# bliunlpr/Robust_e2e_gan

Measured on NVIDIA B200. Metric: utterances/sec (joint step fwd/bwd), higher is better.
Workload: dtype fp32

## Files before the change

robust_e2e_gan_b200/csrc/attloc_loop.cu:

```cuda
#include <math_constants.h>

#include "attloc_common.cuh"
#include "tc_common.cuh"

namespace re2e {
namespace {

#ifdef RE2E_ATT_DEBUG
__device__ long long g_loop_dbg[2][16 * 512];
#define LOOP_DBG_DECL                                                  \
  __shared__ long long dbg_acc[16];                                    \
  if (threadIdx.x == 0)                                                \
    for (int i_ = 0; i_ < 16; ++i_) dbg_acc[i_] = 0;                   \
  long long dbg_last = clock64()
#define LOOP_MARK(slot)                                              \
  do {                                                               \
    if (threadIdx.x == 0) {                                          \
      const long long t_ = clock64();                                \
      dbg_acc[slot] += t_ - dbg_last;                                \
      dbg_last = t_;                                                 \
    }                                                                \
  } while (0)
#define LOOP_DBG_FLUSH(which)                                                                   \
  do {                                                                                          \
    if (threadIdx.x == 0)                                                                       \
      for (int i_ = 0; i_ < 16; ++i_) g_loop_dbg[which][blockIdx.x * 16 + i_] = dbg_acc[i_];    \
  } while (0)
#else
#define LOOP_DBG_DECL
#define LOOP_MARK(slot)
#define LOOP_DBG_FLUSH(which)
#endif

__device__ __forceinline__ void cp_async4(void *dst_smem, const void *src_gmem) {
  asm volatile("cp.async.ca.shared.global [%0], [%1], 4;" ::"r"(smem_u32(dst_smem)), "l"(src_gmem) : "memory");
}
__device__ __forceinline__ void cp_async_commit() { asm volatile("cp.async.commit_group;" ::: "memory"); }
__device__ __forceinline__ void cp_async_wait_all() { asm volatile("cp.async.wait_group 0;" ::: "memory"); }

__device__ __forceinline__ void warp_reduce10(float (&v)[10], int lane) {
  {
    const bool up = lane & 16;
#pragma unroll
    for (int i = 0; i < 5; ++i) {
      const float send = up ? v[i] : v[i + 5], keep = up ? v[i + 5] : v[i];
      v[i] = keep + __shfl_xor_sync(0xffffffffu, send, 16);
    }
  }
  {
    const bool up = lane & 8;
#pragma unroll
    for (int i = 0; i < 2; ++i) {
      const float send = up ? v[i] : v[i + 3], keep = up ? v[i + 3] : v[i];
      v[i] = keep + __shfl_xor_sync(0xffffffffu, send, 8);
    }
    v[2] += __shfl_xor_sync(0xffffffffu, v[2], 8);
  }
  {
    const bool up = lane & 4;
    const float send = up ? v[0] : v[1], keep = up ? v[1] : v[0];
    v[0] = keep + __shfl_xor_sync(0xffffffffu, send, 4);
    v[2] += __shfl_xor_sync(0xffffffffu, v[2], 4);
  }
  {
    const bool up = lane & 2;
    const float send = up ? v[0] : v[2], keep = up ? v[2] : v[0];
    v[0] = keep + __shfl_xor_sync(0xffffffffu, send, 2);
  }
  v[0] += __shfl_xor_sync(0xffffffffu, v[0], 1);
}

constexpr int kLP = 8;
constexpr int kLW = 2 * kLP;
constexpr int kLT = kLW * 32;
constexpr int kLMaxCL = 8;
constexpr int kKG = 12;

struct LoopGeom {
  int tloc_max, App, CKp, Thp, Dp;
  int col_enc, ncols;
};

struct LoopFwdParams {
  const float *pre, *enc, *dec_proj, *att_init, *W_att, *W_conv, *gvec, *gvec_b;
  float scaling;
  float *c_all, *w_all, *conv_all;
  int S, B, Th, D, A, C, K;
  LoopGeom g;
};

struct LoopBwdParams {
  const float *pre, *enc, *dec_proj, *att_init, *w_all, *conv_all, *dc_all, *dw_all, *W_att, *W_conv, *gvec;
  float scaling;
  float *d_pre, *d_decproj, *acc_slots;
  int slot_stride;
  int S, B, Th, D, A, C, K;
  LoopGeom g;
};

template <int APL, int CP, int DPL>
__global__ void __launch_bounds__(kLT, 1) attloc_loop_fwd_kernel(const LoopFwdParams p) {
  constexpr int NT = kLT;
  constexpr int WP = CP + 1;
  constexpr int CPP = (CP + 3) & ~3;
  extern __shared__ __align__(128) unsigned char smraw[];
  const LoopGeom g = p.g;
  const int C = CP == 10 ? 10 : p.C;
  const int Th = p.Th, D = p.D, A = p.A, K = p.K, S = p.S, B = p.B, filts = (p.K - 1) / 2;
  const int tid = threadIdx.x, lane = tid & 31, warp = tid >> 5, half = warp & 1, pair = warp >> 1;
  const int CL = (int)cluster_nctarank(), rank = (int)cluster_ctarank();
  const int b = blockIdx.x / CL;
  const int t0 = min(Th, rank * g.tloc_max), t1 = min(Th, t0 + g.tloc_max), tloc = t1 - t0;
  const int nch = (tloc + kLP - 1) / kLP;
  const int Dp = g.Dp, Dh = (D + 1) / 2;

  uint64_t *full = reinterpret_cast<uint64_t *>(smraw);
  uint64_t *xbar = full + 1;
  uint64_t *tbar = xbar + 2;
  float *tile = reinterpret_cast<float *>(smraw + 128);
  float *app = tile + (size_t)g.tloc_max * (A + D);
  float *wc_s = app + g.App;
  float *watt_s = wc_s + g.CKp;
  float *convp = watt_s + A * WP;
  float *conv_s = convp + round4(kKQ * g.tloc_max * CP);
  float *e_all = conv_s + g.tloc_max * CPP;
  float *epart = e_all + 2 * g.Thp;
  float *cred = epart + round4(2 * g.tloc_max);
  float *cbuf = cred + kLP * Dp;

  const uint32_t xbytes = (uint32_t)Th * 4u + (rank == 0 ? (uint32_t)CL * (uint32_t)D * 4u : 0u);
  if (tid == 0) {
    mbar_init(full, 1);
    mbar_init(&xbar[0], 1);
    mbar_init(&xbar[1], 1);
    mbar_init(tbar, 1);
    mbar_fence_init();
    mbar_expect_tx(&xbar[0], xbytes);
    mbar_expect_tx(&xbar[1], xbytes);
    if (rank == 0) mbar_expect_tx(tbar, (uint32_t)CL * (uint32_t)D * 4u);
  }
  cluster_arrive_relaxed();
  float gv[APL];
#pragma unroll
  for (int j = 0; j < APL; ++j) gv[j] = __ldg(p.gvec + half * (A / 2) + lane + 32 * j);
  const float gb = __ldg(p.gvec_b);
  for (int i = tid; i < C * K; i += NT) wc_s[i] = __ldg(p.W_conv + i);
  for (int i = tid; i < A * C; i += NT) { const int a = i / C; watt_s[a * WP + (i - a * C)] = __ldg(p.W_att + i); }
  pdl_wait();
  if (tid == 0 && tloc > 0) {
    mbar_expect_tx(full, (uint32_t)tloc * (uint32_t)(A + D) * 4u);
    bulk_g2s(tile, p.pre + ((size_t)b * Th + t0) * A, (uint32_t)tloc * A * 4u, full);
    bulk_g2s(tile + (size_t)g.tloc_max * A, p.enc + ((size_t)b * Th + t0) * D, (uint32_t)tloc * D * 4u, full);
  }
  for (int i = tid; i < g.App; i += NT) {
    const int t = i - filts;
    app[i] = (t >= 0 && t < Th) ? __ldg(p.att_init + (size_t)b * Th + t) : 0.0f;
  }
  __syncthreads();
  constexpr int APH = (APL + 1) / 2;
  float2 WattP[APH][CP];
#pragma unroll
  for (int jp = 0; jp < APH; ++jp) {
    const int a0 = half * (A / 2) + lane + 32 * (2 * jp), a1 = a0 + 32;
#pragma unroll
    for (int c = 0; c < CP; ++c)
      WattP[jp][c] = make_float2(c < C ? watt_s[a0 * WP + c] : 0.0f, (c < C && 2 * jp + 1 < APL) ? watt_s[a1 * WP + c] : 0.0f);
  }
  uint32_t dmask = 0;
#pragma unroll
  for (int j = 0; j < DPL; ++j)
    if (lane + 32 * j < Dh && half * Dh + lane + 32 * j < D) dmask |= 1u << j;
  const int aoff = half * (A / 2) + lane;
  cluster_wait();
  if (tloc > 0) mbar_wait(full, 0);
  LOOP_DBG_DECL;
  LOOP_MARK(0);

  for (int s = 0; s < S; ++s) {
    const uint32_t par = (uint32_t)s & 1u, ph = ((uint32_t)s >> 1) & 1u;
    float *e_cur = e_all + par * g.Thp;
    float *cb = cbuf + par * kLMaxCL * Dp;
    float dp[APL];
#pragma unroll
    for (int j = 0; j < APL; ++j) dp[j] = __ldg(p.dec_proj + ((size_t)s * B + b) * A + aoff + 32 * j);

    {
      const int ntg = (tloc + kTG - 1) / kTG;
      const int Kq = (K + kKQ - 1) / kKQ;
      const int nitems = ntg * C * kKQ;
      for (int item = tid; item < nitems; item += NT) {
        const int tg = item % ntg, rest = item / ntg, c = rest % C, kq = rest / C;
        const int k0 = kq * Kq, k1 = min(K, k0 + Kq);
        const float *wr = wc_s + c * K;
        const float *ar = app + t0 + kTG * tg;
        float a0 = 0.f, a1 = 0.f, a2 = 0.f, a3 = 0.f, a4 = 0.f;
        float x0 = ar[k0], x1 = ar[k0 + 1], x2 = ar[k0 + 2], x3 = ar[k0 + 3];
#pragma unroll 5
        for (int k = k0; k < k1; ++k) {
          const float x4 = ar[k + 4], wv2 = wr[k];
          a0 = fmaf(wv2, x0, a0); a1 = fmaf(wv2, x1, a1); a2 = fmaf(wv2, x2, a2);
          a3 = fmaf(wv2, x3, a3); a4 = fmaf(wv2, x4, a4);
          x0 = x1; x1 = x2; x2 = x3; x3 = x4;
        }
        float *o = convp + ((size_t)kq * g.tloc_max + kTG * tg) * CP + c;
        const int nv = min(kTG, tloc - kTG * tg);
        o[0] = a0;
        if (nv > 1) o[CP] = a1;
        if (nv > 2) o[2 * CP] = a2;
        if (nv > 3) o[3 * CP] = a3;
        if (nv > 4) o[4 * CP] = a4;
      }
    }
    __syncthreads();
    LOOP_MARK(1);
    for (int i = tid; i < tloc * CPP; i += NT) {
      const int tl = i / CPP, c = i - tl * CPP;
      float v = 0.0f;
      if (c < C) {
#pragma unroll
        for (int kq = 0; kq < kKQ; ++kq) v += convp[((size_t)kq * g.tloc_max + tl) * CP + c];
        if (p.conv_all) p.conv_all[(((size_t)s * B + b) * Th + t0 + tl) * C + c] = v;
      }
      conv_s[i] = v;
    }
    __syncthreads();
    LOOP_MARK(2);

    float acc[DPL];
#pragma unroll
    for (int j = 0; j < DPL; ++j) acc[j] = 0.0f;
#pragma unroll 2
    for (int q = 0; q < nch; ++q) {
      const int tl = kLP * q + pair;
      if (tl < tloc) {
        const float *cvp = conv_s + tl * CPP;
        float cv[CPP];
#pragma unroll
        for (int c4 = 0; c4 < CPP; c4 += 4) {
          const float4 t4 = *reinterpret_cast<const float4 *>(cvp + c4);
          cv[c4] = t4.x; cv[c4 + 1] = t4.y; cv[c4 + 2] = t4.z; cv[c4 + 3] = t4.w;
        }
        const float *row = tile + (size_t)tl * A + aoff;
        const float pw = app[filts + t0 + tl];
        const float *er = tile + (size_t)g.tloc_max * A + (size_t)tl * D + half * Dh + lane;
        float part = 0.0f;
#pragma unroll
        for (int jp = 0; jp < APH; ++jp) {
          const bool two = 2 * jp + 1 < APL;
          float2 u = make_float2(dp[2 * jp] + row[64 * jp], two ? dp[2 * jp + 1] + row[64 * jp + 32] : 0.0f);
#pragma unroll
          for (int c = 0; c < CP; ++c) u = __ffma2_rn(WattP[jp][c], make_float2(cv[c], cv[c]), u);
          part = fmaf(gv[2 * jp], tanh_ex2(u.x), part);
          if (two) part = fmaf(gv[2 * jp + 1], tanh_ex2(u.y), part);
        }
#pragma unroll
        for (int j = 0; j < DPL; ++j)
          if (dmask & (1u << j)) acc[j] = fmaf(pw, er[32 * j], acc[j]);
        part = warp_sum(part);
        if (lane == 0) epart[2 * tl + half] = part;
      }
    }
#pragma unroll
    for (int j = 0; j < DPL; ++j)
      if (dmask & (1u << j)) cred[pair * Dp + half * Dh + lane + 32 * j] = acc[j];
    LOOP_MARK(3);
    __syncthreads();
    LOOP_MARK(4);

    for (int d = tid; d < D; d += NT) {
      float sum = 0.0f;
#pragma unroll
      for (int pr = 0; pr < kLP; ++pr) sum += cred[pr * Dp + d];
      st_async_f32(dsmem_addr(cb + rank * Dp + d, 0u), s > 0 ? sum : 0.0f, dsmem_addr(&xbar[par], 0u));
    }
    for (int i = tid; i < tloc * CL; i += NT) {
      const int r = i / tloc, tl = i - r * tloc;
      const float e = p.scaling * ((epart[2 * tl] + epart[2 * tl + 1]) + gb);
      st_async_f32(dsmem_addr(e_cur + t0 + tl, (uint32_t)r), e, dsmem_addr(&xbar[par], (uint32_t)r));
    }
    LOOP_MARK(5);
    mbar_wait(&xbar[par], ph);
    LOOP_MARK(6);
    float M = -CUDART_INF_F;
    for (int t = lane; t < Th; t += 32) M = fmaxf(M, e_cur[t]);
    M = warp_max(M);
    float Ssum = 0.0f;
    for (int t = lane; t < Th; t += 32) Ssum += __expf(e_cur[t] - M);
    Ssum = warp_sum(Ssum);
    const float inv = 1.0f / Ssum;
    for (int t = tid; t < Th; t += NT) {
      const float w = __expf(e_cur[t] - M) * inv;
      app[filts + t] = w;
      if (t >= t0 && t < t1) p.w_all[((size_t)s * B + b) * Th + t] = w;
    }
    if (rank == 0 && s > 0) {
      for (int d = tid; d < D; d += NT) {
        float sum = 0.0f;
        for (int r = 0; r < CL; ++r) sum += cb[r * Dp + d];
        p.c_all[((size_t)(s - 1) * B + b) * D + d] = sum;
      }
    }
    if (tid == 0) mbar_expect_tx(&xbar[par], xbytes);
    __syncthreads();
    LOOP_MARK(7);
  }
  {
    float acc[DPL];
#pragma unroll
    for (int j = 0; j < DPL; ++j) acc[j] = 0.0f;
    for (int q = 0; q < nch; ++q) {
      const int tl = kLP * q + pair;
      if (tl < tloc) {
        const float pw = app[filts + t0 + tl];
        const float *er = tile + (size_t)g.tloc_max * A + (size_t)tl * D + half * Dh + lane;
#pragma unroll
        for (int j = 0; j < DPL; ++j)
          if (dmask & (1u << j)) acc[j] = fmaf(pw, er[32 * j], acc[j]);
      }
    }
#pragma unroll
    for (int j = 0; j < DPL; ++j)
      if (dmask & (1u << j)) cred[pair * Dp + half * Dh + lane + 32 * j] = acc[j];
    __syncthreads();
    float *cb = cbuf + ((uint32_t)S & 1u) * kLMaxCL * Dp;
    for (int d = tid; d < D; d += NT) {
      float sum = 0.0f;
#pragma unroll
      for (int pr = 0; pr < kLP; ++pr) sum += cred[pr * Dp + d];
      st_async_f32(dsmem_addr(cb + rank * Dp + d, 0u), sum, dsmem_addr(tbar, 0u));
    }
    if (rank == 0) {
      mbar_wait(tbar, 0);
      for (int d = tid; d < D; d += NT) {
        float sum = 0.0f;
        for (int r = 0; r < CL; ++r) sum += cb[r * Dp + d];
        p.c_all[((size_t)(S - 1) * B + b) * D + d] = sum;
      }
    }
  }
  LOOP_DBG_FLUSH(0);
}

template <int N>
__device__ __forceinline__ void tmem_ldn(uint32_t taddr, float *v);
template <>
__device__ __forceinline__ void tmem_ldn<1>(uint32_t taddr, float *v) {
  uint32_t r0;
  asm volatile("tcgen05.ld.sync.aligned.32x32b.x1.b32 {%0}, [%1];" : "=r"(r0) : "r"(taddr));
  v[0] = __uint_as_float(r0);
}
template <>
__device__ __forceinline__ void tmem_ldn<2>(uint32_t taddr, float *v) {
  uint32_t r0, r1;
  asm volatile("tcgen05.ld.sync.aligned.32x32b.x2.b32 {%0, %1}, [%2];" : "=r"(r0), "=r"(r1) : "r"(taddr));
  v[0] = __uint_as_float(r0); v[1] = __uint_as_float(r1);
}
template <>
__device__ __forceinline__ void tmem_ldn<4>(uint32_t taddr, float *v) {
  uint32_t r0, r1, r2, r3;
  asm volatile("tcgen05.ld.sync.aligned.32x32b.x4.b32 {%0, %1, %2, %3}, [%4];"
               : "=r"(r0), "=r"(r1), "=r"(r2), "=r"(r3) : "r"(taddr));
  v[0] = __uint_as_float(r0); v[1] = __uint_as_float(r1); v[2] = __uint_as_float(r2); v[3] = __uint_as_float(r3);
}
template <>
__device__ __forceinline__ void tmem_ldn<8>(uint32_t taddr, float *v) {
  uint32_t r[8];
  asm volatile("tcgen05.ld.sync.aligned.32x32b.x8.b32 {%0, %1, %2, %3, %4, %5, %6, %7}, [%8];"
               : "=r"(r[0]), "=r"(r[1]), "=r"(r[2]), "=r"(r[3]), "=r"(r[4]), "=r"(r[5]), "=r"(r[6]), "=r"(r[7])
               : "r"(taddr));
#pragma unroll
  for (int i = 0; i < 8; ++i) v[i] = __uint_as_float(r[i]);
}
// ... 46 lines not shown
  constexpr int NT = kLT;
  constexpr int WP = CP + 1;
  constexpr int CPP = (CP + 3) & ~3;
  constexpr int CH2 = (CP + 1) / 2;
  extern __shared__ __align__(128) unsigned char smraw[];
  const LoopGeom g = p.g;
  const int C = CP == 10 ? 10 : p.C;
  const int Th = p.Th, D = p.D, A = p.A, K = p.K, S = p.S, B = p.B, filts = (p.K - 1) / 2;
  const int tid = threadIdx.x, lane = tid & 31, warp = tid >> 5, half = warp & 1, pair = warp >> 1;
  const int CL = (int)cluster_nctarank(), rank = (int)cluster_ctarank();
  const int b = blockIdx.x / CL;
  const int t0 = min(Th, rank * g.tloc_max), t1 = min(Th, t0 + g.tloc_max), tloc = t1 - t0;
  const int nchx = (tloc + kLP - 1) / kLP;
  const int nche = (tloc + kLW - 1) / kLW;
  const int nchx_max = (g.tloc_max + kLP - 1) / kLP, nche_max = (g.tloc_max + kLW - 1) / kLW;

  uint64_t *done_x = reinterpret_cast<uint64_t *>(smraw);
  uint64_t *xbar1 = done_x + 1;
  uint64_t *xbar2 = xbar1 + 2;
  uint32_t *tmem_slot = reinterpret_cast<uint32_t *>(xbar2 + 2);
  float *xs = reinterpret_cast<float *>(smraw + 128);
  float *dcvT = xs + (size_t)g.tloc_max * A;
  float *app = dcvT + 2 * CP * g.App;
  float *wc_s = app + g.App;
  float *conv_s = wc_s + g.CKp;
  float *w_s = conv_s + g.tloc_max * CPP;
  float *dwt_s = w_s + round4(g.tloc_max);
  float *de_s = dwt_s + round4(g.tloc_max);
  float *dwn_s = de_s + round4(g.tloc_max);
  float *dcv_p = dwn_s + round4(g.tloc_max);
  float *ddp_w = dcv_p + 2 * g.tloc_max * 16;
  float *scr = ddp_w + kLW * (A / 2);
  float *ddp_x = scr + max(A * WP, round4(kKQ * CP * g.tloc_max));
  float *xch = ddp_x + 2 * kLMaxCL * A;
  float *slot = p.acc_slots + (size_t)blockIdx.x * p.slot_stride;

  const uint32_t x1bytes = (uint32_t)CL * 4u;
  const uint32_t x2bytes = (uint32_t)Th * (uint32_t)C * 4u + (rank == 0 ? (uint32_t)CL * (uint32_t)A * 4u : 0u);
  if (tid == 0) {
    mbar_init(done_x, kLW);
    for (int i = 0; i < 2; ++i) { mbar_init(&xbar1[i], 1); mbar_init(&xbar2[i], 1); }
    mbar_fence_init();
    for (int i = 0; i < 2; ++i) { mbar_expect_tx(&xbar1[i], x1bytes); mbar_expect_tx(&xbar2[i], x2bytes); }
  }
  cluster_arrive_relaxed();
  if (warp == 0) tmem_alloc(tmem_slot, 512);
  float gv[APL];
#pragma unroll
  for (int j = 0; j < APL; ++j) gv[j] = __ldg(p.gvec + half * (A / 2) + lane + 32 * j);
  for (int i = tid; i < C * K; i += NT) wc_s[i] = __ldg(p.W_conv + i);
  for (int i = tid; i < A * C; i += NT) { const int a = i / C; scr[a * WP + (i - a * C)] = __ldg(p.W_att + i); }
  {
    const int padn = g.App - Th;
    for (int i = tid; i < 2 * CP * padn; i += NT) {
      const int c = i / padn, o = i - c * padn;
      dcvT[c * g.App + (o < filts ? o : Th + o)] = 0.0f;
    }
    for (int i = tid; i < g.tloc_max * CPP; i += NT) conv_s[i] = 0.0f;
    for (int i = tid; i < round4(g.tloc_max); i += NT) dwn_s[i] = 0.0f;
  }
  tc_fence_before();
  __syncthreads();
  tc_fence_after();
  const uint32_t tbase = *tmem_slot + ((uint32_t)(32 * (warp & 3)) << 16);
  const uint32_t tcol_pre = tbase + (uint32_t)((warp >> 2) * nchx_max * APL);
  const uint32_t tcol_enc = tbase + (uint32_t)(g.col_enc + (warp >> 2) * nche_max * DPL2);
  float2 WattC[APL][CH2];
#pragma unroll
  for (int j = 0; j < APL; ++j) {
    const int a = half * (A / 2) + lane + 32 * j;
#pragma unroll
    for (int c2 = 0; c2 < CH2; ++c2)
      WattC[j][c2] = make_float2(2 * c2 < C ? scr[a * WP + 2 * c2] : 0.0f, 2 * c2 + 1 < C ? scr[a * WP + 2 * c2 + 1] : 0.0f);
  }
  const int aoff = half * (A / 2) + lane;
  pdl_wait();
  for (int q = 0; q < nchx; ++q) {
    const int tl = kLP * q + pair;
    float v[APL];
#pragma unroll
    for (int j = 0; j < APL; ++j) v[j] = tl < tloc ? __ldg(p.pre + ((size_t)b * Th + t0 + tl) * A + aoff + 32 * j) : 0.0f;
    tmem_store<APL>(tcol_pre + (uint32_t)(q * APL), v);
  }
  for (int q = 0; q < nche; ++q) {
    const int tl = kLW * q + warp;
    float v[DPL2];
#pragma unroll
    for (int j = 0; j < DPL2; ++j)
      v[j] = (tl < tloc && lane + 32 * j < D) ? __ldg(p.enc + ((size_t)b * Th + t0 + tl) * D + lane + 32 * j) : 0.0f;
    tmem_store<DPL2>(tcol_enc + (uint32_t)(q * DPL2), v);
  }
  tmem_wait_st();
  __syncthreads();
  cluster_wait();

  float pacc[kKG];
#pragma unroll
  for (int i = 0; i < kKG; ++i) pacc[i] = 0.0f;
  float dgv[APL];
#pragma unroll
  for (int j = 0; j < APL; ++j) dgv[j] = 0.0f;
  float dgb = 0.0f;
  const int nkg = (K + kKG - 1) / kKG;
  const bool conv_thread = tid >= A && tid - A < C * nkg;
  const int cw_c = conv_thread ? (tid - A) / nkg : 0, cw_kb = conv_thread ? ((tid - A) % nkg) * kKG : 0;
  LOOP_DBG_DECL;
  LOOP_MARK(0);

  for (int it = 0; it < S; ++it) {
    const int s = S - 1 - it;
    const uint32_t par = (uint32_t)it & 1u, ph = ((uint32_t)it >> 1) & 1u;
    float *dcv_cur = dcvT + par * CP * g.App;
    float *ddpx = ddp_x + par * kLMaxCL * A;
    float *xc = xch + par * kLMaxCL;
    const size_t sb = (size_t)s * B + b;
    float dcr[DPL2];
#pragma unroll
    for (int j = 0; j < DPL2; ++j) dcr[j] = (p.dc_all && lane + 32 * j < D) ? __ldg(p.dc_all + sb * D + lane + 32 * j) : 0.0f;
    float dp[APL];
#pragma unroll
    for (int j = 0; j < APL; ++j) dp[j] = __ldg(p.dec_proj + sb * A + aoff + 32 * j);
    for (int i = tid; i < tloc; i += NT) {
      w_s[i] = __ldg(p.w_all + sb * Th + t0 + i);
      dwt_s[i] = dwn_s[i] + (p.dw_all ? __ldg(p.dw_all + sb * Th + t0 + i) : 0.0f);
    }
    for (int i = tid; i < tloc * C; i += NT) {
      const int tl = i / C;
      conv_s[tl * CPP + (i - tl * C)] = __ldg(p.conv_all + (sb * Th + t0) * C + i);
    }
    {
      const float *prev = s == 0 ? p.att_init + (size_t)b * Th : p.w_all + (sb - B) * Th;
      for (int i = tid; i < g.App; i += NT) {
        const int t = i - filts;
        app[i] = (t >= 0 && t < Th) ? __ldg(prev + t) : 0.0f;
      }
    }
    __syncthreads();
    LOOP_MARK(1);

    for (int q = 0; q < nche; ++q) {
      const int tl = kLW * q + warp;
      float ev[DPL2];
      tmem_load<DPL2>(tcol_enc + (uint32_t)(q * DPL2), ev);
      tmem_wait_ld();
      float dot = 0.0f;
#pragma unroll
      for (int j = 0; j < DPL2; ++j) dot = fmaf(dcr[j], ev[j], dot);
      dot = warp_sum(dot);
      if (lane == 0 && tl < tloc) dwt_s[tl] += dot;
    }
    __syncthreads();
    LOOP_MARK(2);
    if (warp == 0) {
      float s1 = 0.0f;
      for (int tl = lane; tl < tloc; tl += 32) s1 = fmaf(w_s[tl], dwt_s[tl], s1);
      s1 = warp_sum(s1);
      if (lane < CL) st_async_f32(dsmem_addr(xc + rank, (uint32_t)lane), s1, dsmem_addr(&xbar1[par], (uint32_t)lane));
    }
    mbar_wait(&xbar1[par], ph);
    float Stot = 0.0f;
    for (int r = 0; r < CL; ++r) Stot += xc[r];
    for (int tl = tid; tl < tloc; tl += NT) de_s[tl] = p.scaling * w_s[tl] * (dwt_s[tl] - Stot);
    if (tid == 0) {
      mbar_expect_tx(&xbar1[par], x1bytes);
      if (it > 0) bulk_wait<0>();
    }
    __syncthreads();
    LOOP_MARK(3);

    float ddp[APL];
#pragma unroll
    for (int j = 0; j < APL; ++j) ddp[j] = 0.0f;
    float pn[APL];
    tmem_load<APL>(tcol_pre, pn);
#pragma unroll 1
    for (int q = 0; q < nchx; ++q) {
      const int tl = kLP * q + pair;
      tmem_wait_ld();
      float pv[APL];
#pragma unroll
      for (int j = 0; j < APL; ++j) {
        asm volatile("" : "+f"(pn[j]));
        pv[j] = pn[j];
      }
      if (q + 1 < nchx) tmem_load<APL>(tcol_pre + (uint32_t)((q + 1) * APL), pn);
      if (tl < tloc) {
        const float de = de_s[tl];
        const float *cvp = conv_s + tl * CPP;
        float cv[CPP];
#pragma unroll
        for (int c4 = 0; c4 < CPP; c4 += 4) {
// ... 34 lines not shown
#pragma unroll
          for (int c = 0; c < 8; ++c) { dcv[2 * c] = dcv2[c].x; dcv[2 * c + 1] = dcv2[c].y; }
          warp_reduce16(dcv, lane);
          if ((lane & 1) == 0) {
            const int ci = ((lane >> 4) & 1) * 8 + ((lane >> 3) & 1) * 4 + ((lane >> 2) & 1) * 2 + ((lane >> 1) & 1);
            dcv_p[(half * g.tloc_max + tl) * 16 + ci] = dcv[0];
          }
        }
      }
    }
    LOOP_MARK(4);
    fence_proxy_async_smem();
    __syncwarp();
    if (lane == 0) mbar_arrive1(done_x);
    if (tid == 0 && tloc > 0) {
      mbar_wait(done_x, (uint32_t)it & 1u);
      float *dst = p.d_pre + ((size_t)b * Th + t0) * A;
      const uint32_t total = (uint32_t)tloc * A * 4u;
      for (uint32_t o = 0; o < total; o += 32768u) {
        const uint32_t nb = total - o < 32768u ? total - o : 32768u;
        if (it > 0) bulk_red_add_s2g(reinterpret_cast<char *>(dst) + o, reinterpret_cast<char *>(xs) + o, nb);
        else bulk_s2g(reinterpret_cast<char *>(dst) + o, reinterpret_cast<char *>(xs) + o, nb);
      }
      bulk_commit();
    }
#pragma unroll
    for (int j = 0; j < APL; ++j) ddp_w[warp * (A / 2) + lane + 32 * j] = ddp[j];
    __syncthreads();
    LOOP_MARK(5);

    for (int item = tid; item < tloc * C; item += NT) {
      const int c = item / tloc, tl = item - c * tloc;
      const float v = dcv_p[tl * 16 + c] + dcv_p[(g.tloc_max + tl) * 16 + c];
      for (int r = 0; r < CL; ++r)
        st_async_f32(dsmem_addr(dcv_cur + c * g.App + filts + t0 + tl, (uint32_t)r), v, dsmem_addr(&xbar2[par], (uint32_t)r));
    }
    for (int a = tid; a < A; a += NT) {
      const int h = a >= A / 2 ? 1 : 0, ai = a - h * (A / 2);
      float sd = 0.0f;
#pragma unroll
      for (int pr = 0; pr < kLP; ++pr) sd += ddp_w[(2 * pr + h) * (A / 2) + ai];
      st_async_f32(dsmem_addr(ddpx + rank * A + a, 0u), sd, dsmem_addr(&xbar2[par], 0u));
    }
    if (warp == kLW - 1) {
      float s2 = 0.0f;
      for (int tl = lane; tl < tloc; tl += 32) s2 += de_s[tl];
      dgb += warp_sum(s2);
    }
    LOOP_MARK(6);
    if (tid < A) {
#pragma unroll 5
      for (int tl = 0; tl < tloc; ++tl) {
        const float dt = xs[(size_t)tl * A + tid];
#pragma unroll
        for (int c4 = 0; c4 < CPP; c4 += 4) {
          const float4 t4 = *reinterpret_cast<const float4 *>(conv_s + tl * CPP + c4);
          if (c4 < CP) pacc[c4] = fmaf(dt, t4.x, pacc[c4]);
          if (c4 + 1 < CP) pacc[c4 + 1] = fmaf(dt, t4.y, pacc[c4 + 1]);
          if (c4 + 2 < CP) pacc[c4 + 2] = fmaf(dt, t4.z, pacc[c4 + 2]);
          if (c4 + 3 < CP) pacc[c4 + 3] = fmaf(dt, t4.w, pacc[c4 + 3]);
        }
      }
    } else if (conv_thread) {
      const float *ar = app + cw_kb;
      float x[kKG];
#pragma unroll
      for (int i = 0; i < kKG - 1; ++i) x[i] = ar[t0 + i];
#pragma unroll 12
      for (int tl = 0; tl < tloc; ++tl) {
        x[kKG - 1] = ar[t0 + tl + kKG - 1];
        const float dv = dcv_p[tl * 16 + cw_c] + dcv_p[(g.tloc_max + tl) * 16 + cw_c];
#pragma unroll
        for (int i = 0; i < kKG; ++i) pacc[i] = fmaf(dv, x[i], pacc[i]);
#pragma unroll
        for (int i = 0; i < kKG - 1; ++i) x[i] = x[i + 1];
      }
    }
    LOOP_MARK(7);
    mbar_wait(&xbar2[par], ph);
    LOOP_MARK(8);
    if (rank == 0) {
      for (int a = tid; a < A; a += NT) {
        float sd = 0.0f;
        for (int r = 0; r < CL; ++r) sd += ddpx[r * A + a];
        p.d_decproj[sb * A + a] = sd;
      }
    }
    if (s > 0) {
      const int nsg = (tloc + kTG - 1) / kTG;
      const int Kq = (K + kKQ - 1) / kKQ;
      const int nitems = nsg * C * kKQ;
      for (int item = tid; item < nitems; item += NT) {
        const int sg = item % nsg, rest = item / nsg, c = rest % C, kq = rest / C;
        const int k0 = kq * Kq, k1 = min(K, k0 + Kq);
        const float *wr = wc_s + c * K;
        const float *dr = dcv_cur + c * g.App + (t0 + kTG * sg) + 2 * filts;
        float a0 = 0.f, a1 = 0.f, a2 = 0.f, a3 = 0.f, a4 = 0.f;
        float x1 = dr[1 - k0], x2 = dr[2 - k0], x3 = dr[3 - k0], x4 = dr[4 - k0];
#pragma unroll 5
        for (int k = k0; k < k1; ++k) {
          const float x0 = dr[-k], wv = wr[k];
          a0 = fmaf(wv, x0, a0); a1 = fmaf(wv, x1, a1); a2 = fmaf(wv, x2, a2);
          a3 = fmaf(wv, x3, a3); a4 = fmaf(wv, x4, a4);
          x4 = x3; x3 = x2; x2 = x1; x1 = x0;
        }
        float *o = scr + ((size_t)(kq * C + c)) * g.tloc_max + kTG * sg;
        const int nv = min(kTG, tloc - kTG * sg);
        o[0] = a0;
        if (nv > 1) o[1] = a1;
        if (nv > 2) o[2] = a2;
        if (nv > 3) o[3] = a3;
        if (nv > 4) o[4] = a4;
      }
    }
    if (tid == 0) mbar_expect_tx(&xbar2[par], x2bytes);
    __syncthreads();
    LOOP_MARK(9);
    if (s > 0) {
      for (int tl = tid; tl < tloc; tl += NT) {
        float sum = 0.0f;
        for (int i = 0; i < kKQ * C; ++i) sum += scr[(size_t)i * g.tloc_max + tl];
        dwn_s[tl] = sum;
      }
    }
    LOOP_MARK(10);
  }

  LOOP_DBG_FLUSH(1);
  if (tid < A) {
#pragma unroll
    for (int c = 0; c < CP; ++c)
      if (c < C) slot[tid * C + c] = pacc[c];
  } else if (conv_thread) {
#pragma unroll
    for (int i = 0; i < kKG; ++i)
      if (cw_kb + i < K) slot[A * C + cw_c * K + cw_kb + i] = pacc[i];
  }
  __syncthreads();
#pragma unroll
  for (int j = 0; j < APL; ++j) ddp_w[warp * (A / 2) + lane + 32 * j] = dgv[j];
  __syncthreads();
  for (int a = tid; a < A; a += NT) {
    const int h = a >= A / 2 ? 1 : 0, ai = a - h * (A / 2);
    float sg = 0.0f;
#pragma unroll
    for (int pr = 0; pr < kLP; ++pr) sg += ddp_w[(2 * pr + h) * (A / 2) + ai];
    slot[A * C + C * K + a] = sg;
  }
  if (warp == kLW - 1 && lane == 0) slot[A * C + C * K + A] = dgb;
  if (tid == 0) bulk_wait<0>();
  tc_fence_before();
  __syncthreads();
  if (warp == 0) tmem_dealloc(*tmem_slot, 512);
}

inline int loop_check_dims(int S, int B, int Th, int D, int A, int C, int K) {
  if (S <= 0 || B <= 0 || Th <= 0 || D <= 0 || A <= 0 || C <= 0 || K <= 0) return RE2E_E_ARG;
  if ((K & 1) == 0) return RE2E_E_ARG;
  if (A % 64 != 0 || A > 512 || (D & 3) || D > 512 || C > 16) return RE2E_E_UNSUPPORTED;
  const int apl = A / 64;
  if (!(apl == 1 || apl == 2 || apl == 4 || apl == 5 || apl == 8)) return RE2E_E_UNSUPPORTED;
  return RE2E_OK;
}

inline int pick_cl(int B, int Th) {
  const int sms = num_sms();
  int CL = 1;
  while (CL < kLMaxCL && B * CL * 2 <= sms) CL *= 2;
  while (CL > 1 && (Th + CL - 1) / CL < kLP) CL /= 2;
  return CL;
}

inline void loop_geom_common(int Th, int D, int C, int K, int CL, LoopGeom &g) {
  const int filts = (K - 1) / 2;
  g.tloc_max = (Th + CL - 1) / CL;
  g.App = round4(Th + 2 * filts + 8);
  g.CKp = round4(C * K);
  g.Thp = round4(Th);
  g.Dp = round4(D);
  g.col_enc = 0;
  g.ncols = 0;
}

inline bool loop_geom_fwd(int B, int Th, int D, int A, int C, int K, int CP, int &CL, LoopGeom &g, size_t &smem) {
  CL = pick_cl(B, Th);
  const int CPP = round4(CP);
  for (;;) {
    loop_geom_common(Th, D, C, K, CL, g);
    const size_t floats = (size_t)g.tloc_max * (A + D) + g.App + g.CKp + (size_t)A * (CP + 1) +
                          round4(kKQ * g.tloc_max * CP) + (size_t)g.tloc_max * CPP + 2 * (size_t)g.Thp +
                          round4(g.tloc_max) + round4(2 * g.tloc_max) + 2 * kLW + (size_t)kLP * g.Dp +
                          2 * (size_t)kLMaxCL * g.Dp + 4 * kLMaxCL;
    smem = 128 + sizeof(float) * floats;
    if (smem <= 226 * 1024) return true;
    if (CL >= kLMaxCL || B * CL * 2 > num_sms()) return false;
    CL *= 2;
  }
}

inline bool loop_geom_bwd(int B, int Th, int D, int A, int C, int K, int CP, int dpl2, int &CL, LoopGeom &g,
                          size_t &smem) {
  CL = pick_cl(B, Th);
  const int CPP = round4(CP);
  const int nkg = (K + kKG - 1) / kKG;
  if (A + C * nkg > kLT) return false;
  for (;;) {
    loop_geom_common(Th, D, C, K, CL, g);
    const int nchx_max = (g.tloc_max + kLP - 1) / kLP, nche_max = (g.tloc_max + kLW - 1) / kLW;
    g.col_enc = 4 * nchx_max * (A / 64);
    g.ncols = g.col_enc + 4 * nche_max * dpl2;
    const size_t scr = (size_t)A * (CP + 1) > (size_t)round4(kKQ * CP * g.tloc_max) ? (size_t)A * (CP + 1)
                                                                                   : (size_t)round4(kKQ * CP * g.tloc_max);
    const size_t floats = (size_t)g.tloc_max * A + 2 * (size_t)CP * g.App + g.App + g.CKp + (size_t)g.tloc_max * CPP +
                          4 * (size_t)round4(g.tloc_max) + 2 * (size_t)g.tloc_max * 16 + (size_t)kLW * (A / 2) + scr +
                          2 * (size_t)kLMaxCL * A + 2 * kLMaxCL;
    smem = 128 + sizeof(float) * floats;
    if (smem <= 226 * 1024 && g.ncols <= 512) return true;
    if (CL >= kLMaxCL || B * CL * 2 > num_sms()) return false;
    CL *= 2;
  }
}

template <typename Kern, typename Params>
int launch_loop(Kern kern, const Params &prm, int B, int CL, size_t smem, cudaStream_t st) {
  int rc0 = ensure_smem(reinterpret_cast<const void *>(kern), smem);
  if (rc0 != RE2E_OK) return rc0;
  cudaLaunchConfig_t cfg{};
  cfg.gridDim = dim3((unsigned)(B * CL));
  cfg.blockDim = dim3((unsigned)kLT);
  cfg.dynamicSmemBytes = smem;
  cfg.stream = st;
  cudaLaunchAttribute attr[2];
  attr[0].id = cudaLaunchAttributeClusterDimension;
  attr[0].val.clusterDim.x = (unsigned)CL;
  attr[0].val.clusterDim.y = 1;
  attr[0].val.clusterDim.z = 1;
  attr[1].id = cudaLaunchAttributeProgrammaticStreamSerialization;
  attr[1].val.programmaticStreamSerializationAllowed = 1;
  cfg.attrs = attr;
  cfg.numAttrs = 2;
  cudaError_t e = cudaLaunchKernelEx(&cfg, kern, prm);
  count_launch();
  return e == cudaSuccess ? RE2E_OK : (int)e;
}

#define LOOP_DISPATCH(NAME, APLV, CPV, ...)                                             \
  switch (APLV) {                                                                       \
    case 1: rc = (CPV) == 10 ? NAME<1, 10> __VA_ARGS__ : NAME<1, 16> __VA_ARGS__; break; \
    case 2: rc = (CPV) == 10 ? NAME<2, 10> __VA_ARGS__ : NAME<2, 16> __VA_ARGS__; break; \
    case 4: rc = (CPV) == 10 ? NAME<4, 10> __VA_ARGS__ : NAME<4, 16> __VA_ARGS__; break; \
    case 5: rc = (CPV) == 10 ? NAME<5, 10> __VA_ARGS__ : NAME<5, 16> __VA_ARGS__; break; \
    case 8: rc = (CPV) == 10 ? NAME<8, 10> __VA_ARGS__ : NAME<8, 16> __VA_ARGS__; break; \
    default: rc = RE2E_E_UNSUPPORTED;                                                   \
  }

template <int APL, int CP>
int run_loop_fwd(const LoopFwdParams &prm, int CL, size_t smem, cudaStream_t st) {
  if (prm.D == prm.A) return launch_loop(attloc_loop_fwd_kernel<APL, CP, APL>, prm, prm.B, CL, smem, st);
  return launch_loop(attloc_loop_fwd_kernel<APL, CP, 8>, prm, prm.B, CL, smem, st);
}
template <int APL, int CP>
int run_loop_bwd(const LoopBwdParams &prm, int CL, size_t smem, cudaStream_t st) {
  if (prm.D == prm.A) return launch_loop(attloc_loop_bwd_kernel<APL, CP, 2 * APL>, prm, prm.B, CL, smem, st);
  return launch_loop(attloc_loop_bwd_kernel<APL, CP, 16>, prm, prm.B, CL, smem, st);
}

}
}

using namespace re2e;

#ifdef RE2E_ATT_DEBUG
extern "C" int re2e_loop_debug_read(long long *host_out, int which) {
  cudaDeviceSynchronize();
  return (int)cudaMemcpyFromSymbol(host_out, g_loop_dbg, sizeof(long long) * 16 * 512, sizeof(long long) * 16 * 512 * which);
}
#endif

extern "C" int re2e_attloc_loop_supported(int S, int B, int Th, int D, int A, int C, int K) {
  int rc = loop_check_dims(S, B, Th, D, A, C, K);
  if (rc != RE2E_OK) return 0;
  const int CP = C == 10 ? 10 : 16;
  int CLf, CLb;
  size_t smem;
  LoopGeom g;
  if (!loop_geom_fwd(B, Th, D, A, C, K, CP, CLf, g, smem)) return 0;
  if (!loop_geom_bwd(B, Th, D, A, C, K, CP, D == A ? 2 * (A / 64) : 16, CLb, g, smem)) return 0;
  return 1;
}

extern "C" int re2e_attloc_loop_slots(int S, int B, int Th, int D, int A, int C, int K) {
  int rc = loop_check_dims(S, B, Th, D, A, C, K);
// ... 57 lines not shown
```

Before: 24870.

## Defer attention context to batched post-loop GEMM and distribute reductions across cluster

The forward loop no longer computes the per-step context vector inside the sequential decoder loop. It instead computes all contexts after the loop in blocks of steps, using packed FMA over re-read attention weights, and reduces across the cluster through DSMEM with the output split by rank. The backward pass precomputes the encoder·dc dot for the next step so it overlaps with the cross-CTA exchange. It also spreads the d_decproj reduction across ranks instead of rank 0, and uses float2 FMA accumulators plus a named barrier. Shared-memory layout and geometry constraints change, which adds complexity and more cluster syncs in the context phase.

```diff
diff --git a/robust_e2e_gan_b200/csrc/attloc_loop.cu b/robust_e2e_gan_b200/csrc/attloc_loop.cu
--- a/robust_e2e_gan_b200/csrc/attloc_loop.cu
+++ b/robust_e2e_gan_b200/csrc/attloc_loop.cu
@@ -37,6 +37,12 @@
 }
 __device__ __forceinline__ void cp_async_commit() { asm volatile("cp.async.commit_group;" ::: "memory"); }
 __device__ __forceinline__ void cp_async_wait_all() { asm volatile("cp.async.wait_group 0;" ::: "memory"); }
+__device__ __forceinline__ float4 dsmem_ld4(uint32_t addr) {
+  float4 v;
+  asm volatile("ld.shared::cluster.v4.f32 {%0, %1, %2, %3}, [%4];" : "=f"(v.x), "=f"(v.y), "=f"(v.z), "=f"(v.w) : "r"(addr)
+               : "memory");
+  return v;
+}
 
 __device__ __forceinline__ void warp_reduce10(float (&v)[10], int lane) {
   {
@@ -75,6 +81,9 @@
 constexpr int kLT = kLW * 32;
 constexpr int kLMaxCL = 8;
 constexpr int kKG = 12;
+constexpr int kCtxSB = 24;
+constexpr int kCtxMaxSB = 48;
+constexpr int kCtxSG = 4;
 
 struct LoopGeom {
   int tloc_max, App, CKp, Thp, Dp;
@@ -98,7 +107,7 @@
   LoopGeom g;
 };
 
-template <int APL, int CP, int DPL>
+template <int APL, int CP>
 __global__ void __launch_bounds__(kLT, 1) attloc_loop_fwd_kernel(const LoopFwdParams p) {
   constexpr int NT = kLT;
   constexpr int WP = CP + 1;
@@ -112,11 +121,10 @@
   const int b = blockIdx.x / CL;
   const int t0 = min(Th, rank * g.tloc_max), t1 = min(Th, t0 + g.tloc_max), tloc = t1 - t0;
   const int nch = (tloc + kLP - 1) / kLP;
-  const int Dp = g.Dp, Dh = (D + 1) / 2;
+  const int Dp = g.Dp;
 
   uint64_t *full = reinterpret_cast<uint64_t *>(smraw);
   uint64_t *xbar = full + 1;
-  uint64_t *tbar = xbar + 2;
   float *tile = reinterpret_cast<float *>(smraw + 128);
   float *app = tile + (size_t)g.tloc_max * (A + D);
   float *wc_s = app + g.App;
@@ -125,19 +133,16 @@
   float *conv_s = convp + round4(kKQ * g.tloc_max * CP);
   float *e_all = conv_s + g.tloc_max * CPP;
   float *epart = e_all + 2 * g.Thp;
-  float *cred = epart + round4(2 * g.tloc_max);
-  float *cbuf = cred + kLP * Dp;
-
-  const uint32_t xbytes = (uint32_t)Th * 4u + (rank == 0 ? (uint32_t)CL * (uint32_t)D * 4u : 0u);
+  float *cpart = epart + round4(2 * g.tloc_max);
+
+  const uint32_t xbytes = (uint32_t)Th * 4u;
   if (tid == 0) {
     mbar_init(full, 1);
     mbar_init(&xbar[0], 1);
     mbar_init(&xbar[1], 1);
-    mbar_init(tbar, 1);
     mbar_fence_init();
     mbar_expect_tx(&xbar[0], xbytes);
     mbar_expect_tx(&xbar[1], xbytes);
-    if (rank == 0) mbar_expect_tx(tbar, (uint32_t)CL * (uint32_t)D * 4u);
   }
   cluster_arrive_relaxed();
   float gv[APL];
@@ -166,10 +171,6 @@
     for (int c = 0; c < CP; ++c)
       WattP[jp][c] = make_float2(c < C ? watt_s[a0 * WP + c] : 0.0f, (c < C && 2 * jp + 1 < APL) ? watt_s[a1 * WP + c] : 0.0f);
   }
-  uint32_t dmask = 0;
-#pragma unroll
-  for (int j = 0; j < DPL; ++j)
-    if (lane + 32 * j < Dh && half * Dh + lane + 32 * j < D) dmask |= 1u << j;
   const int aoff = half * (A / 2) + lane;
   cluster_wait();
   if (tloc > 0) mbar_wait(full, 0);
@@ -179,7 +180,6 @@
   for (int s = 0; s < S; ++s) {
     const uint32_t par = (uint32_t)s & 1u, ph = ((uint32_t)s >> 1) & 1u;
     float *e_cur = e_all + par * g.Thp;
-    float *cb = cbuf + par * kLMaxCL * Dp;
     float dp[APL];
 #pragma unroll
     for (int j = 0; j < APL; ++j) dp[j] = __ldg(p.dec_proj + ((size_t)s * B + b) * A + aoff + 32 * j);
@@ -226,9 +226,6 @@
     __syncthreads();
     LOOP_MARK(2);
 
-    float acc[DPL];
-#pragma unroll
-    for (int j = 0; j < DPL; ++j) acc[j] = 0.0f;
 #pragma unroll 2
     for (int q = 0; q < nch; ++q) {
       const int tl = kLP * q + pair;
@@ -241,8 +238,6 @@
           cv[c4] = t4.x; cv[c4 + 1] = t4.y; cv[c4 + 2] = t4.z; cv[c4 + 3] = t4.w;
         }
         const float *row = tile + (size_t)tl * A + aoff;
-        const float pw = app[filts + t0 + tl];
-        const float *er = tile + (size_t)g.tloc_max * A + (size_t)tl * D + half * Dh + lane;
         float part = 0.0f;
 #pragma unroll
         for (int jp = 0; jp < APH; ++jp) {
@@ -253,26 +248,14 @@
           part = fmaf(gv[2 * jp], tanh_ex2(u.x), part);
           if (two) part = fmaf(gv[2 * jp + 1], tanh_ex2(u.y), part);
         }
-#pragma unroll
-        for (int j = 0; j < DPL; ++j)
-          if (dmask & (1u << j)) acc[j] = fmaf(pw, er[32 * j], acc[j]);
         part = warp_sum(part);
         if (lane == 0) epart[2 * tl + half] = part;
       }
     }
-#pragma unroll
-    for (int j = 0; j < DPL; ++j)
-      if (dmask & (1u << j)) cred[pair * Dp + half * Dh + lane + 32 * j] = acc[j];
     LOOP_MARK(3);
     __syncthreads();
     LOOP_MARK(4);
 
-    for (int d = tid; d < D; d += NT) {
-      float sum = 0.0f;
-#pragma unroll
-      for (int pr = 0; pr < kLP; ++pr) sum += cred[pr * Dp + d];
-      st_async_f32(dsmem_addr(cb + rank * Dp + d, 0u), s > 0 ? sum : 0.0f, dsmem_addr(&xbar[par], 0u));
-    }
     for (int i = tid; i < tloc * CL; i += NT) {
       const int r = i / tloc, tl = i - r * tloc;
       const float e = p.scaling * ((epart[2 * tl] + epart[2 * tl + 1]) + gb);
@@ -293,51 +276,63 @@
       app[filts + t] = w;
       if (t >= t0 && t < t1) p.w_all[((size_t)s * B + b) * Th + t] = w;
     }
-    if (rank == 0 && s > 0) {
-      for (int d = tid; d < D; d += NT) {
-        float sum = 0.0f;
-        for (int r = 0; r < CL; ++r) sum += cb[r * Dp + d];
-        p.c_all[((size_t)(s - 1) * B + b) * D + d] = sum;
-      }
-    }
     if (tid == 0) mbar_expect_tx(&xbar[par], xbytes);
     __syncthreads();
     LOOP_MARK(7);
   }
   {
-    float acc[DPL];
-#pragma unroll
-    for (int j = 0; j < DPL; ++j) acc[j] = 0.0f;
-    for (int q = 0; q < nch; ++q) {
-      const int tl = kLP * q + pair;
-      if (tl < tloc) {
-        const float pw = app[filts + t0 + tl];
-        const float *er = tile + (size_t)g.tloc_max * A + (size_t)tl * D + half * Dh + lane;
-#pragma unroll
-        for (int j = 0; j < DPL; ++j)
-          if (dmask & (1u << j)) acc[j] = fmaf(pw, er[32 * j], acc[j]);
-      }
-    }
-#pragma unroll
-    for (int j = 0; j < DPL; ++j)
-      if (dmask & (1u << j)) cred[pair * Dp + half * Dh + lane + 32 * j] = acc[j];
-    __syncthreads();
-    float *cb = cbuf + ((uint32_t)S & 1u) * kLMaxCL * Dp;
-    for (int d = tid; d < D; d += NT) {
-      float sum = 0.0f;
-#pragma unroll
-      for (int pr = 0; pr < kLP; ++pr) sum += cred[pr * Dp + d];
-      st_async_f32(dsmem_addr(cb + rank * Dp + d, 0u), sum, dsmem_addr(tbar, 0u));
-    }
-    if (rank == 0) {
-      mbar_wait(tbar, 0);
-      for (int d = tid; d < D; d += NT) {
-        float sum = 0.0f;
-        for (int r = 0; r < CL; ++r) sum += cb[r * Dp + d];
-        p.c_all[((size_t)(S - 1) * B + b) * D + d] = sum;
-      }
-    }
-  }
+    const int sb_pre = min(kCtxMaxSB, (g.tloc_max * A / Dp) & ~(kCtxSG - 1));
+    float *cp = sb_pre > kCtxSB ? tile : cpart;
+    const int SB = max(sb_pre, kCtxSB);
+    const int D4 = D / 4, nsg = SB / kCtxSG;
+    const int Dsl4 = (D4 + CL - 1) / CL;
+    float *ws = convp;
+    for (int s0 = 0; s0 < S; s0 += SB) {
+      const int nsb = min(SB, S - s0);
+      for (int i = tid; i < nsb * tloc; i += NT) {
+        const int sl = i / tloc, tl = i - sl * tloc;
+        ws[sl * g.tloc_max + tl] = p.w_all[((size_t)(s0 + sl) * B + b) * Th + t0 + tl];
+      }
+      __syncthreads();
+      for (int item = tid; item < D4 * nsg; item += NT) {
+        const int d4 = item % D4, sg = item / D4;
+        if (sg * kCtxSG >= nsb) continue;
+        float2 lo[kCtxSG], hi[kCtxSG];
+#pragma unroll
+        for (int i = 0; i < kCtxSG; ++i) { lo[i] = make_float2(0.0f, 0.0f); hi[i] = lo[i]; }
+        const float *er = tile + (size_t)g.tloc_max * A + 4 * d4;
+        const float *wr = ws + sg * kCtxSG * g.tloc_max;
+#pragma unroll 2
+        for (int tl = 0; tl < tloc; ++tl) {
+          const float4 e4 = *reinterpret_cast<const float4 *>(er + (size_t)tl * D);
+          const float2 elo = make_float2(e4.x, e4.y), ehi = make_float2(e4.z, e4.w);
+#pragma unroll
+          for (int i = 0; i < kCtxSG; ++i) {
+            const float w = wr[i * g.tloc_max + tl];
+            lo[i] = __ffma2_rn(make_float2(w, w), elo, lo[i]);
+            hi[i] = __ffma2_rn(make_float2(w, w), ehi, hi[i]);
+          }
+        }
+#pragma unroll
+        for (int i = 0; i < kCtxSG; ++i)
+          *reinterpret_cast<float4 *>(cp + (sg * kCtxSG + i) * Dp + 4 * d4) = make_float4(lo[i].x, lo[i].y, hi[i].x, hi[i].y);
+      }
+      cluster_sync_all();
+      for (int item = tid; item < nsb * Dsl4; item += NT) {
+        const int sl = item / Dsl4, d4 = rank * Dsl4 + (item - sl * Dsl4);
+        if (d4 >= D4) continue;
+        const uint32_t off = (uint32_t)((sl * Dp + 4 * d4) * 4);
+        float4 sum = make_float4(0.0f, 0.0f, 0.0f, 0.0f);
+        for (int r = 0; r < CL; ++r) {
+          const float4 v = dsmem_ld4(dsmem_addr(cp, (uint32_t)r) + off);
+          sum.x += v.x; sum.y += v.y; sum.z += v.z; sum.w += v.w;
+        }
+        *reinterpret_cast<float4 *>(p.c_all + ((size_t)(s0 + sl) * B + b) * D + 4 * d4) = sum;
+      }
+      cluster_sync_all();
+    }
+  }
+  LOOP_MARK(8);
   LOOP_DBG_FLUSH(0);
 }
 
@@ -450,11 +445,13 @@
   float *ddp_w = dcv_p + 2 * g.tloc_max * 16;
   float *scr = ddp_w + kLW * (A / 2);
   float *ddp_x = scr + max(A * WP, round4(kKQ * CP * g.tloc_max));
+  float *edc = ddp_x + 2 * A;
   float *xch = ddp_x + 2 * kLMaxCL * A;
   float *slot = p.acc_slots + (size_t)blockIdx.x * p.slot_stride;
 
   const uint32_t x1bytes = (uint32_t)CL * 4u;
-  const uint32_t x2bytes = (uint32_t)Th * (uint32_t)C * 4u + (rank == 0 ? (uint32_t)CL * (uint32_t)A * 4u : 0u);
+  const int Asl = A / CL;
+  const uint32_t x2bytes = (uint32_t)Th * (uint32_t)C * 4u + (uint32_t)A * 4u;
   if (tid == 0) {
     mbar_init(done_x, kLW);
     for (int i = 0; i < 2; ++i) { mbar_init(&xbar1[i], 1); mbar_init(&xbar2[i], 1); }
@@ -509,12 +506,36 @@
     tmem_store<DPL2>(tcol_enc + (uint32_t)(q * DPL2), v);
   }
   tmem_wait_st();
+  float dcr[DPL2];
+  auto load_dc = [&](int s) {
+#pragma unroll
+    for (int j = 0; j < DPL2; ++j)
+      dcr[j] = lane + 32 * j < D ? __ldg(p.dc_all + ((size_t)s * B + b) * D + lane + 32 * j) : 0.0f;
+  };
+  auto enc_dot_dc = [&]() {
+    for (int q = 0; q < nche; ++q) {
+      const int tl = kLW * q + warp;
+      float ev[DPL2];
+      tmem_load<DPL2>(tcol_enc + (uint32_t)(q * DPL2), ev);
+      tmem_wait_ld();
+      float dot = 0.0f;
+#pragma unroll
+      for (int j = 0; j < DPL2; ++j) dot = fmaf(dcr[j], ev[j], dot);
+      dot = warp_sum(dot);
+      if (lane == 0 && tl < tloc) edc[tl] = dot;
+    }
+  };
+  if (p.dc_all) {
+    load_dc(S - 1);
+    enc_dot_dc();
+  }
   __syncthreads();
   cluster_wait();
 
-  float pacc[kKG];
-#pragma unroll
-  for (int i = 0; i < kKG; ++i) pacc[i] = 0.0f;
+  constexpr int NACC2 = (CP > kKG ? CP : kKG) / 2;
+  float2 pacc[NACC2];
+#pragma unroll
+  for (int i = 0; i < NACC2; ++i) pacc[i] = make_float2(0.0f, 0.0f);
   float dgv[APL];
 #pragma unroll
   for (int j = 0; j < APL; ++j) dgv[j] = 0.0f;
@@ -529,18 +550,17 @@
     const int s = S - 1 - it;
     const uint32_t par = (uint32_t)it & 1u, ph = ((uint32_t)it >> 1) & 1u;
     float *dcv_cur = dcvT + par * CP * g.App;
-    float *ddpx = ddp_x + par * kLMaxCL * A;
+    float *ddpx = ddp_x + par * A;
     float *xc = xch + par * kLMaxCL;
     const size_t sb = (size_t)s * B + b;
-    float dcr[DPL2];
-#pragma unroll
-    for (int j = 0; j < DPL2; ++j) dcr[j] = (p.dc_all && lane + 32 * j < D) ? __ldg(p.dc_all + sb * D + lane + 32 * j) : 0.0f;
     float dp[APL];
 #pragma unroll
     for (int j = 0; j < APL; ++j) dp[j] = __ldg(p.dec_proj + sb * A + aoff + 32 * j);
     for (int i = tid; i < tloc; i += NT) {
       w_s[i] = __ldg(p.w_all + sb * Th + t0 + i);
-      dwt_s[i] = dwn_s[i] + (p.dw_all ? __ldg(p.dw_all + sb * Th + t0 + i) : 0.0f);
+      float v = dwn_s[i] + (p.dw_all ? __ldg(p.dw_all + sb * Th + t0 + i) : 0.0f);
+      if (p.dc_all) v += edc[i];
+      dwt_s[i] = v;
     }
     for (int i = tid; i < tloc * C; i += NT) {
       const int tl = i / C;
@@ -555,26 +575,17 @@
     }
     __syncthreads();
     LOOP_MARK(1);
-
-    for (int q = 0; q < nche; ++q) {
-      const int tl = kLW * q + warp;
-      float ev[DPL2];
-      tmem_load<DPL2>(tcol_enc + (uint32_t)(q * DPL2), ev);
-      tmem_wait_ld();
-      float dot = 0.0f;
-#pragma unroll
-      for (int j = 0; j < DPL2; ++j) dot = fmaf(dcr[j], ev[j], dot);
-      dot = warp_sum(dot);
-      if (lane == 0 && tl < tloc) dwt_s[tl] += dot;
-    }
-    __syncthreads();
-    LOOP_MARK(2);
     if (warp == 0) {
       float s1 = 0.0f;
       for (int tl = lane; tl < tloc; tl += 32) s1 = fmaf(w_s[tl], dwt_s[tl], s1);
       s1 = warp_sum(s1);
       if (lane < CL) st_async_f32(dsmem_addr(xc + rank, (uint32_t)lane), s1, dsmem_addr(&xbar1[par], (uint32_t)lane));
     }
+    if (p.dc_all && s > 0) {
+      load_dc(s - 1);
+      enc_dot_dc();
+    }
+    LOOP_MARK(2);
     mbar_wait(&xbar1[par], ph);
     float Stot = 0.0f;
     for (int r = 0; r < CL; ++r) Stot += xc[r];
@@ -675,6 +686,7 @@
     for (int item = tid; item < tloc * C; item += NT) {
       const int c = item / tloc, tl = item - c * tloc;
       const float v = dcv_p[tl * 16 + c] + dcv_p[(g.tloc_max + tl) * 16 + c];
+      dcv_p[tl * 16 + c] = v;
       for (int r = 0; r < CL; ++r)
         st_async_f32(dsmem_addr(dcv_cur + c * g.App + filts + t0 + tl, (uint32_t)r), v, dsmem_addr(&xbar2[par], (uint32_t)r));
     }
@@ -683,7 +695,8 @@
       float sd = 0.0f;
 #pragma unroll
       for (int pr = 0; pr < kLP; ++pr) sd += ddp_w[(2 * pr + h) * (A / 2) + ai];
-      st_async_f32(dsmem_addr(ddpx + rank * A + a, 0u), sd, dsmem_addr(&xbar2[par], 0u));
+      const int ro = a / Asl;
+      st_async_f32(dsmem_addr(ddpx + rank * Asl + (a - ro * Asl), (uint32_t)ro), sd, dsmem_addr(&xbar2[par], (uint32_t)ro));
     }
     if (warp == kLW - 1) {
       float s2 = 0.0f;
@@ -691,17 +704,18 @@
       dgb += warp_sum(s2);
     }
     LOOP_MARK(6);
+    if (tid < A) asm volatile("bar.arrive 1, %0;" ::"r"(NT) : "memory");
+    else asm volatile("bar.sync 1, %0;" ::"r"(NT) : "memory");
     if (tid < A) {
 #pragma unroll 5
       for (int tl = 0; tl < tloc; ++tl) {
         const float dt = xs[(size_t)tl * A + tid];
+        const float2 dt2 = make_float2(dt, dt);
 #pragma unroll
         for (int c4 = 0; c4 < CPP; c4 += 4) {
           const float4 t4 = *reinterpret_cast<const float4 *>(conv_s + tl * CPP + c4);
-          if (c4 < CP) pacc[c4] = fmaf(dt, t4.x, pacc[c4]);
-          if (c4 + 1 < CP) pacc[c4 + 1] = fmaf(dt, t4.y, pacc[c4 + 1]);
-          if (c4 + 2 < CP) pacc[c4 + 2] = fmaf(dt, t4.z, pacc[c4 + 2]);
-          if (c4 + 3 < CP) pacc[c4 + 3] = fmaf(dt, t4.w, pacc[c4 + 3]);
+          if (c4 < CP) pacc[c4 / 2] = __ffma2_rn(dt2, make_float2(t4.x, t4.y), pacc[c4 / 2]);
+          if (c4 + 2 < CP) pacc[c4 / 2 + 1] = __ffma2_rn(dt2, make_float2(t4.z, t4.w), pacc[c4 / 2 + 1]);
         }
       }
     } else if (conv_thread) {
@@ -712,9 +726,12 @@
 #pragma unroll 12
       for (int tl = 0; tl < tloc; ++tl) {
         x[kKG - 1] = ar[t0 + tl + kKG - 1];
-        const float dv = dcv_p[tl * 16 + cw_c] + dcv_p[(g.tloc_max + tl) * 16 + cw_c];
-#pragma unroll
-        for (int i = 0; i < kKG; ++i) pacc[i] = fmaf(dv, x[i], pacc[i]);
+        const float dv = dcv_p[tl * 16 + cw_c];
+#pragma unroll
+        for (int i = 0; i < kKG / 2; ++i) {
+          pacc[i].x = fmaf(dv, x[2 * i], pacc[i].x);
+          pacc[i].y = fmaf(dv, x[2 * i + 1], pacc[i].y);
+        }
 #pragma unroll
         for (int i = 0; i < kKG - 1; ++i) x[i] = x[i + 1];
       }
@@ -722,12 +739,10 @@
     LOOP_MARK(7);
     mbar_wait(&xbar2[par], ph);
     LOOP_MARK(8);
-    if (rank == 0) {
-      for (int a = tid; a < A; a += NT) {
-        float sd = 0.0f;
-        for (int r = 0; r < CL; ++r) sd += ddpx[r * A + a];
-        p.d_decproj[sb * A + a] = sd;
-      }
+    for (int a = tid; a < Asl; a += NT) {
+      float sd = 0.0f;
+      for (int r = 0; r < CL; ++r) sd += ddpx[r * Asl + a];
+      p.d_decproj[sb * A + rank * Asl + a] = sd;
     }
     if (s > 0) {
       const int nsg = (tloc + kTG - 1) / kTG;
@@ -773,11 +788,11 @@
   if (tid < A) {
 #pragma unroll
     for (int c = 0; c < CP; ++c)
-      if (c < C) slot[tid * C + c] = pacc[c];
+      if (c < C) slot[tid * C + c] = c & 1 ? pacc[c / 2].y : pacc[c / 2].x;
   } else if (conv_thread) {
 #pragma unroll
     for (int i = 0; i < kKG; ++i)
-      if (cw_kb + i < K) slot[A * C + cw_c * K + cw_kb + i] = pacc[i];
+      if (cw_kb + i < K) slot[A * C + cw_c * K + cw_kb + i] = i & 1 ? pacc[i / 2].y : pacc[i / 2].x;
   }
   __syncthreads();
 #pragma unroll
@@ -832,8 +847,8 @@
     loop_geom_common(Th, D, C, K, CL, g);
     const size_t floats = (size_t)g.tloc_max * (A + D) + g.App + g.CKp + (size_t)A * (CP + 1) +
                           round4(kKQ * g.tloc_max * CP) + (size_t)g.tloc_max * CPP + 2 * (size_t)g.Thp +
-                          round4(g.tloc_max) + round4(2 * g.tloc_max) + 2 * kLW + (size_t)kLP * g.Dp +
-                          2 * (size_t)kLMaxCL * g.Dp + 4 * kLMaxCL;
+                          round4(g.tloc_max) + round4(2 * g.tloc_max) + 2 * kLW + (size_t)kCtxSB * g.Dp +
+                          4 * kLMaxCL;
     smem = 128 + sizeof(float) * floats;
     if (smem <= 226 * 1024) return true;
     if (CL >= kLMaxCL || B * CL * 2 > num_sms()) return false;
@@ -858,7 +873,7 @@
                           4 * (size_t)round4(g.tloc_max) + 2 * (size_t)g.tloc_max * 16 + (size_t)kLW * (A / 2) + scr +
                           2 * (size_t)kLMaxCL * A + 2 * kLMaxCL;
     smem = 128 + sizeof(float) * floats;
-    if (smem <= 226 * 1024 && g.ncols <= 512) return true;
+    if (smem <= 226 * 1024 && g.ncols <= 512 && round4(g.tloc_max) <= (2 * kLMaxCL - 2) * A) return true;
     if (CL >= kLMaxCL || B * CL * 2 > num_sms()) return false;
     CL *= 2;
   }
@@ -899,8 +914,7 @@
 
 template <int APL, int CP>
 int run_loop_fwd(const LoopFwdParams &prm, int CL, size_t smem, cudaStream_t st) {
-  if (prm.D == prm.A) return launch_loop(attloc_loop_fwd_kernel<APL, CP, APL>, prm, prm.B, CL, smem, st);
-  return launch_loop(attloc_loop_fwd_kernel<APL, CP, 8>, prm, prm.B, CL, smem, st);
+  return launch_loop(attloc_loop_fwd_kernel<APL, CP>, prm, prm.B, CL, smem, st);
 }
 template <int APL, int CP>
 int run_loop_bwd(const LoopBwdParams &prm, int CL, size_t smem, cudaStream_t st) {
```

After: 25150, median of 6. +1.1%, better.
